# IlzeAmandaA/VAE-GP-ODE

Measured on AMD Instinct MI355X. Metric: latent_trajectories_per_sec, higher is better.
Workload: dtype f32; 1 GPU; configs[1]: ode1 DF q=6 M=100 S=256 T=16 batch=256; step = full ELBO training step (encoder, GP draw, rk4 rollout, decoder, ELBO, backward, Adam), L=1; global_batch=256, mc_draws=1, solver=rk4 (3/8 rule), parallelism=dp1, hip_graph=True, graph_scope=whole, gp_side_stream=True, batchnorm=per-process statistics

## Files before the change

vae-gp-ode_amd/csrc/conv_mfma.hpp:

```cpp
#pragma once
#include <hip/hip_runtime.h>
#include <cstdint>
#include <type_traits>
#include "bn_math.hpp"
#include "bn_sink.hpp"

namespace gp {

typedef float f32x4 __attribute__((ext_vector_type(4)));

template <int N, class F> __device__ __forceinline__ void static_for(F&& f) {
  if constexpr (N > 0) {
    static_for<N - 1>(f);
    f(std::integral_constant<int, N - 1>{});
  }
}

#ifdef CONVT_PROBE
__device__ unsigned long long g_probe[8];
#define PROBE_T(v) const long long v = clock64()
#define PROBE_ADD(i, v) do { if (threadIdx.x == 0 && blockIdx.x == 0) g_probe[i] += (unsigned long long)(clock64() - (v)); } while (0)
#else
#define PROBE_T(v)
#define PROBE_ADD(i, v)
#endif

constexpr int cmax_(int a, int b) { return a > b ? a : b; }
constexpr int plane_stride_unit(int n) { return ((n + 15) / 32) * 32 + 16; }

template <class L, int NCS_> struct FwdPolicy {
  static constexpr int KC = L::CI, NC = L::CO, NCS = NCS_, NCLS = L::S * L::S, KK = L::K * L::K;
  static constexpr int SH = L::HI, OH = L::HO, HP = L::HP, PADL = L::PL;
  static constexpr int PS = plane_stride_unit(HP * HP);
  static constexpr int WROW = NCS;
  static constexpr int WSLAB = KK * KC * WROW;
  static constexpr int NWE = KC * NCS * KK;
  static constexpr int class_tap_offset(int cls) {
    int off = 0;
    for (int c = 0; c < cls; ++c) off += ((L::K - c / L::S + L::S - 1) / L::S) * ((L::K - c % L::S + L::S - 1) / L::S);
    return off;
  }
  template <int CLS> struct C {
    static constexpr int py = CLS / L::S, px = CLS % L::S;
    static constexpr int nty = (L::K - py + L::S - 1) / L::S, ntx = (L::K - px + L::S - 1) / L::S, ntaps = nty * ntx;
    static constexpr int qy0 = cmax_(0, (L::P - py + L::S - 1) / L::S), qx0 = cmax_(0, (L::P - px + L::S - 1) / L::S);
    static constexpr int ny = (L::HO - 1 + L::P - py) / L::S - qy0 + 1, nx = (L::HO - 1 + L::P - px) / L::S - qx0 + 1;
    static constexpr int npc = ny * nx;
    static constexpr int slab_taps = class_tap_offset(CLS);
    static __device__ __forceinline__ int tap_off(int t) { return -(t / ntx) * HP - t % ntx; }
    static __device__ __forceinline__ int pix_addr(int p) { return (qy0 + p / nx + PADL) * HP + qx0 + p % nx + PADL; }
    static constexpr __host__ __device__ int out_off(int p) {
      return (L::S * (qy0 + p / nx) + py - L::P) * OH + L::S * (qx0 + p % nx) + px - L::P;
    }
  };
  static __device__ __forceinline__ size_t w_src(int e, int n0) {
    const int ci = e / (NCS * KK), r = e % (NCS * KK);
    return ((size_t)ci * NC + n0) * KK + r;
  }
  static __device__ __forceinline__ int w_dst(int e) {
    const int ci = e / (NCS * KK), r = e % (NCS * KK), col = r / KK, ky = (r % KK) / L::K, kx = r % L::K;
    const int py = ky % L::S, px = kx % L::S;
    int off = 0;
    for (int c = 0; c < py * L::S + px; ++c) off += ((L::K - c / L::S + L::S - 1) / L::S) * ((L::K - c % L::S + L::S - 1) / L::S);
    const int tap = (ky / L::S) * ((L::K - px + L::S - 1) / L::S) + kx / L::S;
    return ((off + tap) * KC + ci) * WROW + col;
  }
};

template <class L, int NCS_> struct BwdDataPolicy {
  static constexpr int KC = L::CO, NC = L::CI, NCS = NCS_, NCLS = 1, KK = L::K * L::K;
  static constexpr int SH = L::HO, OH = L::HI, HP = L::GP_, PADL = L::P;
  static constexpr int PS = L::S == 1 ? plane_stride_unit(HP * HP) : (HP * HP) | 1;
  static constexpr int WROW = NCS;
  static constexpr int WSLAB = KK * KC * WROW;
  static constexpr int NWE = KC * NCS * KK;
  template <int CLS> struct C {
    static constexpr int ntaps = KK, ntx = L::K, npc = L::HI * L::HI, nx = L::HI, slab_taps = 0;
    static __device__ __forceinline__ int tap_off(int t) { return (t / L::K) * HP + t % L::K; }
    static __device__ __forceinline__ int pix_addr(int p) { return L::S * (p / nx) * HP + L::S * (p % nx); }
    static constexpr __host__ __device__ int out_off(int p) { return p; }
  };
  static __device__ __forceinline__ size_t w_src(int e, int n0) { return (size_t)n0 * KC * KK + e; }
  static __device__ __forceinline__ int w_dst(int e) {
    const int cil = e / (KC * KK), co = (e / KK) % KC, tap = e % KK;
    return (tap * KC + co) * WROW + cil;
  }
};

template <class PL> constexpr bool igemm_tf_in_pad() { return PL::PS % 4 == 0 && (PL::HP * PL::HP + 3) / 4 * 4 + 4 <= PL::PS; }

template <class CG, int NG, int TG, int NCJ, int KC, int WROW, int PS, int KBMAX = 8>
__device__ __forceinline__ void igemm_tile_mma(const float* __restrict__ s_img, const float* __restrict__ sw, const int (&abase)[TG],
                                               int lk, int lr, f32x4 (&acc)[TG][NCJ]) {
  constexpr int KB = (KC / 4) < KBMAX ? (KC / 4) : KBMAX;
  constexpr int NB = KC / (4 * KB);
  constexpr int nsteps = CG::ntaps * NB;
  float bfA[KB][NCJ], afA[KB][NG], bfB[KB][NCJ], afB[KB][NG];
  auto fetch = [&](int s, float (&bf)[KB][NCJ], float (&af)[KB][NG]) {
    const int t = s / NB, cb = (s % NB) * 4 * KB;
    const float* wp = sw + ((size_t)t * KC + cb + lk) * WROW + lr;
    const int ao = CG::tap_off(t) + cb * PS;
#pragma unroll
    for (int kk = 0; kk < KB; ++kk) {
#pragma unroll
      for (int c = 0; c < NCJ; ++c) bf[kk][c] = wp[4 * kk * WROW + c * 16];
#pragma unroll
      for (int g = 0; g < NG; ++g) af[kk][g] = s_img[abase[g] + ao + 4 * kk * PS];
    }
  };
  auto mma = [&](const float (&bf)[KB][NCJ], const float (&af)[KB][NG]) {
#pragma unroll
    for (int kk = 0; kk < KB; ++kk)
#pragma unroll
      for (int g = 0; g < NG; ++g)
#pragma unroll
        for (int c = 0; c < NCJ; ++c)
          acc[g][c] = __builtin_amdgcn_mfma_f32_16x16x4f32(bf[kk][c], af[kk][g], acc[g][c], 0, 0, 0);
  };
  fetch(0, bfA, afA);
  int s = 0;
  if constexpr (KBMAX < 8) {
#pragma nounroll
    while (true) {
      if (s + 1 < nsteps) fetch(s + 1, bfB, afB);
      mma(bfA, afA);
      if (++s >= nsteps) break;
      if (s + 1 < nsteps) fetch(s + 1, bfA, afA);
      mma(bfB, afB);
      if (++s >= nsteps) break;
    }
  } else {
    while (true) {
      if (s + 1 < nsteps) fetch(s + 1, bfB, afB);
      mma(bfA, afA);
      if (++s >= nsteps) break;
      if (s + 1 < nsteps) fetch(s + 1, bfA, afA);
      mma(bfB, afB);
      if (++s >= nsteps) break;
    }
  }
}

extern __shared__ __attribute__((aligned(16))) float igemm_smem[];

template <class PL, int IPB, int TG, int NCJ, bool PAIR, int NTHR, bool DB = false, bool PC = false, bool STATS = false>
__global__ __launch_bounds__(NTHR, NTHR == 256 ? 2 : 1) void k_conv_igemm(const float* __restrict__ x, const float* __restrict__ w,
                                                      const float* __restrict__ bias, float* __restrict__ y, int B,
                                                      const float* __restrict__ in_bn, BnSink sink) {
  constexpr int KC = PL::KC, NC = PL::NC, NCS = PL::NCS, NCLS = PL::NCLS, SH = PL::SH, OH = PL::OH, HP = PL::HP, PS = PL::PS;
  constexpr int PADL = PL::PADL, WROW = PL::WROW, NWE = PL::NWE;
  static_assert(NCS % 16 == 0 && NC % NCS == 0 && KC % 4 == 0 && NTHR % 256 == 0, "MFMA tiling");
  static_assert(!PC || (NTHR == 768 && DB), "producer / consumer form: 8 + 4 wavefronts on double-buffered planes");
  constexpr int NW = PC ? 8 : NTHR / 64;
  constexpr int PT = PC ? 256 : NTHR;
  constexpr int KBM = PC ? 4 : 8;
  constexpr int NCO = NCS / 16;
  static_assert(NCO % NCJ == 0, "channel tiles per job");
  constexpr int NJ = NCO / NCJ;
  static_assert(NJ == 1 || TG == 1, "tile groups share all channel tiles");
  static_assert(!STATS || NJ == 1, "output statistics: a lane keeps the same channels in every job of a pass");
  constexpr int IMG = KC * PS;
  static_assert(IMG % 4 == 0, "float4 zero fill");
  constexpr int SRC = KC * SH * SH;
  static_assert(SRC % 4 == 0, "float4 source fetch");
  constexpr int NLD = (IPB * SRC / 4 + PT - 1) / PT;
  constexpr int NBUF = DB ? 2 : 1;
  float* s_img = igemm_smem;
  float* s_w = igemm_smem + NBUF * IPB * IMG;
  constexpr int TFO = (HP * HP + 3) / 4 * 4;
  constexpr bool TF_PAD = igemm_tf_in_pad<PL>();
  float* s_sm = s_w + PL::WSLAB + (TF_PAD ? 0 : 4 * KC);
  float4* s_tf_tail = reinterpret_cast<float4*>(s_w + PL::WSLAB);
  auto tf_slot = [&](int ch) -> float4* { return TF_PAD ? reinterpret_cast<float4*>(s_img + ch * PS + TFO) : s_tf_tail + ch; };
  const int tid = threadIdx.x, lane = tid & 63, wave = __builtin_amdgcn_readfirstlane(tid >> 6);
  const int lr = lane & 15, lk = lane >> 4;
  const int ptid = PC ? tid - 512 : tid;
  const int ngroups = (B + IPB - 1) / IPB;
  const float4* x4 = reinterpret_cast<const float4*>(x);
  const int jw = (wave & 3) * (NW / 4) + (wave >> 2);

  PROBE_T(pt_all);
  for (int e = tid; e < NBUF * IPB * IMG / 4; e += NTHR) reinterpret_cast<float4*>(s_img)[e] = float4{0.f, 0.f, 0.f, 0.f};
  if (in_bn) {
    if (TF_PAD) __syncthreads();
    for (int e = tid; e < KC; e += NTHR) *tf_slot(e) = reinterpret_cast<const float4*>(in_bn)[e];
  }
  if (STATS)
    for (int e = tid; e < 2 * NC; e += NTHR) s_sm[e] = 0.f;

  constexpr int NPASS = NC / NCS;
  const bool spread = NPASS > 1 && gridDim.x % NPASS == 0;
  const int gstride = spread ? gridDim.x / NPASS : gridDim.x;
  const int gfirst = spread ? blockIdx.x % gstride : blockIdx.x;
  for (int pass = spread ? blockIdx.x / gstride : 0; pass < (spread ? blockIdx.x / gstride + 1 : NPASS); ++pass) {
    const int n0 = pass * NCS;
    __syncthreads();
    PROBE_T(pt_w);
    for (int base = 0; base < NWE; base += NTHR * 8) {
      float v[8];
#pragma unroll
      for (int u = 0; u < 8; ++u) {
        const int e = base + tid + NTHR * u;
        v[u] = e < NWE ? w[PL::w_src(e, n0)] : 0.f;
      }
#pragma unroll
      for (int u = 0; u < 8; ++u) {
        const int e = base + tid + NTHR * u;
        if (e < NWE) s_w[PL::w_dst(e)] = v[u];
      }
    }
    PROBE_ADD(0, pt_w);

    float kshift[NCJ][4], bs[NCJ][4], bq[NCJ][4];
#pragma unroll
    for (int cc = 0; cc < NCJ; ++cc)
#pragma unroll
      for (int r = 0; r < 4; ++r) {
        kshift[cc][r] = STATS ? bn_sink_shift(sink, n0 + cc * 16 + 4 * lk + r) : 0.f;
        bs[cc][r] = bq[cc][r] = 0.f;
      }
    float4 pre[NLD];
    auto prefetch = [&](int grp) __attribute__((always_inline)) {
      const int b0 = grp * IPB;
      const int nf4 = min(IPB, B - b0) * (SRC / 4);
      const float4* src = x4 + (size_t)b0 * (SRC / 4);
#pragma unroll
      for (int i = 0; i < NLD; ++i) {
        const int f = ptid + PT * i;
        if (PC) pre[i] = src[min(f, nf4 - 1)];
        else if (f < nf4) pre[i] = src[f];
      }
    };
    auto scatter = [&](float* __restrict__ img, int nimg) __attribute__((always_inline)) {
      const int nf4 = nimg * (SRC / 4);
#pragma unroll
      for (int i = 0; i < NLD; ++i) {
        const int f = ptid + PT * i;
        if (f < nf4) {
          const float v[4] = {pre[i].x, pre[i].y, pre[i].z, pre[i].w};
          int pl = (4 * f) / (SH * SH), q = (4 * f) % (SH * SH), row = q / SH, col = q % SH;
#pragma unroll
          for (int k = 0; k < 4; ++k) {
            img[pl * PS + (row + PADL) * HP + col + PADL] = in_bn ? bn_relu(v[k], *tf_slot(pl % KC)) : v[k];
            if (SH % 4 != 0 || k < 3) {
              if (++col == SH) { col = 0; if (++row == SH) { row = 0; ++pl; } }
            }
          }
        }
      }
    };
    auto jobs = [&](const float* __restrict__ img, int b0, int nimg, int pf_grp = -1) {
      PROBE_T(pt_rng);
      int wtot = 0;
      constexpr int NCG = PAIR ? NCLS / 2 : NCLS;
      static_for<NCG>([&](auto c) {
        constexpr int c0 = PAIR ? 2 * decltype(c)::value : decltype(c)::value;
        using G0 = typename PL::template C<c0>;
        using G1 = typename PL::template C<PAIR ? c0 + 1 : c0>;
        wtot += ((nimg * G0::npc + 15) / 16) * NJ * (G0::ntaps + (PAIR ? G1::ntaps : 0));
      });
      const int lo = (wtot * jw) / NW, hi = (wtot * (jw + 1)) / NW;
      int cbase = 0;
      PROBE_ADD(0, pt_rng);
      static_for<NCG>([&](auto c) {
        constexpr int c0 = PAIR ? 2 * decltype(c)::value : decltype(c)::value;
        using G = typename PL::template C<c0>;
        using G1 = typename PL::template C<PAIR ? c0 + 1 : c0>;
        static_assert(!PAIR || (G::npc == G1::npc && G::nx == G1::nx), "paired classes cover the same pixel grid");
        static_assert(!PAIR || (G::out_off(0) == G1::out_off(0) + 1 && G::out_off(G::npc - 1) == G1::out_off(G::npc - 1) + 1 &&
                                G1::out_off(0) % 2 == 0 && OH % 2 == 0), "paired classes write neighbouring, 8-byte aligned columns");
        constexpr int ntaps = G::ntaps + (PAIR ? G1::ntaps : 0), npc = G::npc;
        const float* swc = s_w + G::slab_taps * KC * WROW;
        const float* swc1 = s_w + G1::slab_taps * KC * WROW;
        const int mtot = nimg * npc;
        const int njobs = ((mtot + 15) / 16) * NJ;
        const int nlo = lo - cbase - ntaps / 2, nhi = hi - cbase - ntaps / 2;
        const int ub = min(njobs, nlo <= 0 ? 0 : (nlo + ntaps - 1) / ntaps), ue = min(njobs, nhi <= 0 ? 0 : (nhi + ntaps - 1) / ntaps);
        cbase += njobs * ntaps;
        for (int u0 = ub; u0 < ue; u0 += TG) {
          PROBE_T(pt_su);
          const int ng = min(TG, ue - u0);
          const int t0 = u0 / NJ, jc = u0 % NJ;
          int abase[TG], abase1[TG];
#pragma unroll
          for (int g = 0; g < TG; ++g) {
            int m = (t0 + g) * 16 + lr;
            m = (g < ng && m < mtot) ? m : 0;
            const int im = m / npc, p = m % npc;
            abase[g] = im * IMG + lk * PS + G::pix_addr(p);
            abase1[g] = im * IMG + lk * PS + G1::pix_addr(p);
          }
          f32x4 acc[TG][NCJ], acc1[TG][NCJ];
#pragma unroll
          for (int g = 0; g < TG; ++g)
#pragma unroll
            for (int cc = 0; cc < NCJ; ++cc) acc[g][cc] = acc1[g][cc] = f32x4{0.f, 0.f, 0.f, 0.f};
          float bv[NCJ][4];
#pragma unroll
          for (int cc = 0; cc < NCJ; ++cc)
#pragma unroll
            for (int r = 0; r < 4; ++r) bv[cc][r] = bias ? bias[n0 + (jc * NCJ + cc) * 16 + 4 * lk + r] : 0.f;
          PROBE_ADD(6, pt_su);
          PROBE_T(pt_mm);
          auto run = [&](auto gtag, const float* sw, const int (&ab)[TG], f32x4 (&ac)[TG][NCJ]) {
            using GG = typename decltype(gtag)::type;
            switch (ng) {
              case 1: igemm_tile_mma<GG, 1, TG, NCJ, KC, WROW, PS, KBM>(img, sw, ab, lk, lr, ac); break;
              case 2: if constexpr (TG >= 2) igemm_tile_mma<GG, 2, TG, NCJ, KC, WROW, PS, KBM>(img, sw, ab, lk, lr, ac); break;
              case 3: if constexpr (TG >= 3) igemm_tile_mma<GG, 3, TG, NCJ, KC, WROW, PS, KBM>(img, sw, ab, lk, lr, ac); break;
              default: if constexpr (TG >= 4) igemm_tile_mma<GG, 4, TG, NCJ, KC, WROW, PS, KBM>(img, sw, ab, lk, lr, ac); break;
            }
          };
          run(std::common_type<G>{}, swc + jc * NCJ * 16, abase, acc);
          if (pf_grp >= 0) { prefetch(pf_grp); pf_grp = -1; }
          if constexpr (PAIR) run(std::common_type<G1>{}, swc1 + jc * NCJ * 16, abase1, acc1);
          PROBE_ADD(3, pt_mm);
          PROBE_T(pt_st);
#pragma unroll
          for (int g = 0; g < TG; ++g) {
            const int m = (t0 + g) * 16 + lr;
            if (g < ng && m < mtot) {
              const int im = m / npc, p = m % npc;
              const int ch0 = n0 + jc * NCJ * 16 + 4 * lk;
              float* yp = y + ((size_t)(b0 + im) * NC + ch0) * (OH * OH) + (PAIR ? G1::out_off(p) : G::out_off(p));
#pragma unroll
              for (int cc = 0; cc < NCJ; ++cc)
#pragma unroll
                for (int r = 0; r < 4; ++r) {
                  const float v0 = acc[g][cc][r] + bv[cc][r];
                  if constexpr (PAIR) {
                    const float v1 = acc1[g][cc][r] + bv[cc][r];
                    *reinterpret_cast<float2*>(yp + (size_t)(cc * 16 + r) * (OH * OH)) = float2{v1, v0};
                    if (STATS) { const float d = v1 - kshift[cc][r]; bs[cc][r] += d; bq[cc][r] = fmaf(d, d, bq[cc][r]); }
                  } else {
                    yp[(size_t)(cc * 16 + r) * (OH * OH)] = v0;
                  }
                  if (STATS) { const float d = v0 - kshift[cc][r]; bs[cc][r] += d; bq[cc][r] = fmaf(d, d, bq[cc][r]); }
                }
            }
          }
          PROBE_ADD(4, pt_st);
        }
      });
      if (pf_grp >= 0) prefetch(pf_grp);
    };
    if constexpr (PC) {
      const bool producer = wave >= 8;
      int cur = 0;
      if (producer) {
        __builtin_amdgcn_s_setprio(3);
        if (gfirst < ngroups) prefetch(gfirst);
      }
      __syncthreads();
      if (producer) {
        if (gfirst < ngroups) scatter(s_img, min(IPB, B - gfirst * IPB));
        if (gfirst + gstride < ngroups) prefetch(gfirst + gstride);
      }
      __syncthreads();
      for (int grp = gfirst; grp < ngroups; grp += gstride) {
        const int b0 = grp * IPB, nxt = grp + gstride;
        if (producer) {
          if (nxt < ngroups) {
            scatter(s_img + (cur ^ 1) * (IPB * IMG), min(IPB, B - nxt * IPB));
            if (nxt + gstride < ngroups) prefetch(nxt + gstride);
          }
        } else {
          jobs(s_img + cur * (IPB * IMG), b0, min(IPB, B - b0));
        }
        __syncthreads();
        cur ^= 1;
      }
    } else if constexpr (!DB) {
      if (gfirst < ngroups) prefetch(gfirst);
      for (int grp = gfirst; grp < ngroups; grp += gstride) {
        const int b0 = grp * IPB;
        const int nimg = min(IPB, B - b0);
        PROBE_T(pt_b1);
        __syncthreads();
        PROBE_ADD(1, pt_b1);
        PROBE_T(pt_sc);
        scatter(s_img, nimg);
        __syncthreads();
        PROBE_ADD(2, pt_sc);
        PROBE_T(pt_pf);
        PROBE_ADD(7, pt_pf);
        jobs(s_img, b0, nimg, grp + gstride < ngroups ? grp + gstride : -1);
      }
    } else {
      const bool early = wave < NW / 2;
      int cur = 0;
      if (gfirst < ngroups) prefetch(gfirst);
      __syncthreads();
      if (gfirst < ngroups) scatter(s_img, min(IPB, B - gfirst * IPB));
      if (gfirst + gstride < ngroups) prefetch(gfirst + gstride);
      __syncthreads();
      for (int grp = gfirst; grp < ngroups; grp += gstride) {
        const int b0 = grp * IPB, nxt = grp + gstride;
        const int nimg = min(IPB, B - b0);
        float* bc = s_img + cur * (IPB * IMG);
        float* bn = s_img + (cur ^ 1) * (IPB * IMG);
        if (early && nxt < ngroups) {
          scatter(bn, min(IPB, B - nxt * IPB));
          if (nxt + gstride < ngroups) prefetch(nxt + gstride);
        }
        jobs(bc, b0, nimg);
        if (!early && nxt < ngroups) {
          scatter(bn, min(IPB, B - nxt * IPB));
          if (nxt + gstride < ngroups) prefetch(nxt + gstride);
        }
        __syncthreads();
        cur ^= 1;
      }
    }
    if constexpr (STATS) {
      __syncthreads();
      float* red = s_w;
#pragma unroll
      for (int cc = 0; cc < NCJ; ++cc)
#pragma unroll
        for (int r = 0; r < 4; ++r) {
          const float a = row_allreduce16(bs[cc][r]), b = row_allreduce16(bq[cc][r]);
          if (lr == 0 && wave < NW) {
            red[(wave * NCS + cc * 16 + 4 * lk + r) * 2] = a;
            red[(wave * NCS + cc * 16 + 4 * lk + r) * 2 + 1] = b;
          }
        }
      __syncthreads();
      if (tid < 2 * NCS) {
        float t = 0.f;
        for (int wv = 0; wv < NW; ++wv) t += red[wv * NCS * 2 + tid];
        s_sm[2 * n0 + tid] = t;
      }
    }
  }
  if constexpr (STATS) {
    __syncthreads();
    bn_sink_publish<NC, NTHR>(sink, s_sm);
  }
  PROBE_ADD(5, pt_all);
}

constexpr int pad2mod4(int n) { return n + ((2 - n % 4) + 4) % 4; }

template <class L> struct WgradGeo {
  static constexpr int NPIX = L::HI * L::HI, NKS = (NPIX + 3) / 4;
  static constexpr int PSX = pad2mod4(NKS * 4);
  static constexpr int GP = L::GP_;
  static constexpr int GPH = L::S == 2 ? (GP + 1) / 2 : GP;
  static constexpr int HPL = GP * GPH;
  static constexpr int PSG = pad2mod4(L::S == 2 ? 2 * HPL : HPL);
  static constexpr int IMGX = L::CI * PSX, IMGG = L::CO * PSG;
  static_assert(L::S == 1 || L::S == 2, "stride");
};

template <class L, int IPB, int WM, int WN, int WT, bool PIPE, bool HAS_BN, int NTHR>
// ... 206 lines not shown
```

vae-gp-ode_amd/csrc/vae_conv_tiled.hip:

```cpp
#include <hip/hip_runtime.h>
#include <cstdlib>
#include <cstdint>
#include "gp_launch.hpp"
#include <type_traits>
#include "conv_layers.hpp"
#include "conv_mfma.hpp"
#include "conv_dec10_mfma.hpp"
#include "conv_dec1_mfma.hpp"
#include "conv_dec4_mfma.hpp"

namespace gp {



extern __shared__ __attribute__((aligned(16))) float tsm[];

template <class L, int IPB>
__global__ __launch_bounds__(256) void k_convT_fwd(const float* __restrict__ x, const float* __restrict__ w,
                                                    const float* __restrict__ bias, float* __restrict__ y, int B) {
  constexpr int CI = L::CI, CO = L::CO, HI = L::HI, HO = L::HO, HP = L::HP, K = L::K, S = L::S, P = L::P, PL = L::PL;
  constexpr int CPT = CO % 16 == 0 ? 16 : 8;
  static_assert(CO % CPT == 0, "8 or 16 output channels per thread");
  constexpr int NG = CO / CPT;
  constexpr int IMG = CI * HP * HP;
// ... 219 lines not shown
    const int ox0 = seg * 4;
    float acc[4] = {bv, bv, bv, bv};
    const float* img = s_img + im * IMG;
#pragma unroll 2
    for (int ci = 0; ci < CI; ++ci) {
#pragma unroll
      for (int ky = 0; ky < 5; ++ky) {
        const float4* rp = reinterpret_cast<const float4*>(img + (ci * WP + (oy + 4 - ky)) * WP + ox0);
        const float4 a = rp[0], b = rp[1];
        const float v[8] = {a.x, a.y, a.z, a.w, b.x, b.y, b.z, b.w};
        const float4 w4 = *reinterpret_cast<const float4*>(s_w + (ci * 5 + ky) * 8);
        const float w5 = s_w[(ci * 5 + ky) * 8 + 4];
        const float wk[5] = {w4.x, w4.y, w4.z, w4.w, w5};
#pragma unroll
        for (int j = 0; j < 4; ++j)
#pragma unroll
          for (int kx = 0; kx < 5; ++kx) acc[j] = fmaf(v[j + 4 - kx], wk[kx], acc[j]);
      }
    }
    *reinterpret_cast<float4*>(y + ((size_t)(b0 + im) * H + oy) * H + ox0) = make_float4(acc[0], acc[1], acc[2], acc[3]);
  }
}

__global__ __launch_bounds__(256) void k_dec10_wgrad(const float* __restrict__ x, const float* __restrict__ gy,
                                                      float* __restrict__ part, int B, int b_per_split) {
  constexpr int CI = 16, H = 28, NP = H * H, XS = NP + 1, GW = 32;
  float* s_x = tsm;
  float* s_g = tsm + CI * XS;
  const int tid = threadIdx.x, ci = tid & 15, pl = tid >> 4;
  const int b0 = blockIdx.x * b_per_split, b1 = min(B, b0 + b_per_split);
  float acc[25];
#pragma unroll
  for (int t = 0; t < 25; ++t) acc[t] = 0.f;
  for (int b = b0; b < b1; ++b) {
    __syncthreads();
    for (int e = tid; e < CI * NP; e += 256) s_x[(e / NP) * XS + e % NP] = x[(size_t)b * CI * NP + e];
    for (int e = tid; e < GW * GW; e += 256) {
      const int yy = e / GW - 2, xx = e % GW - 2;
      s_g[e] = (yy >= 0 && yy < H && xx >= 0 && xx < H) ? gy[(size_t)b * NP + yy * H + xx] : 0.f;
    }
    __syncthreads();
    for (int p = pl; p < NP; p += 16) {
      const int iy = p / H, ix = p % H;
      const float xv = s_x[ci * XS + p];
      const float* gp = s_g + iy * GW + ix;
#pragma unroll
      for (int ky = 0; ky < 5; ++ky)
#pragma unroll
        for (int kx = 0; kx < 5; ++kx) acc[ky * 5 + kx] = fmaf(xv, gp[ky * GW + kx], acc[ky * 5 + kx]);
    }
  }
  __syncthreads();
  float* s_red = tsm;
#pragma unroll
  for (int t = 0; t < 25; ++t) s_red[(pl * 16 + ci) * 25 + t] = acc[t];
  __syncthreads();
  for (int e = tid; e < CI * 25; e += 256) {
    float v = 0.f;
    for (int l = 0; l < 16; ++l) v += s_red[l * 400 + e];
    part[(size_t)blockIdx.x * 400 + e] = v;
  }
}

__global__ void k_sum_splits_t(const float* __restrict__ part, int nsplit, size_t n, float* __restrict__ out) {
  const size_t e = (size_t)blockIdx.x * blockDim.x + threadIdx.x;
  if (e >= n) return;
  float acc = 0.f;
  for (int s = 0; s < nsplit; ++s) acc += part[(size_t)s * n + e];
  out[e] = acc;
}

template <class L> static bool matches(int Ci_conv, int Co_conv, int H, int Ho, int K, int S, int P) {
  return Ci_conv == L::CO && Co_conv == L::CI && H == L::HO && Ho == L::HI && K == L::K && S == L::S && P == L::P;
}

static bool use_mfma() {
  static int v = -1;
  if (v < 0) { const char* e = getenv("GPODE_CONV_VALU"); v = (e && e[0] == '1') ? 0 : 1; }
  return v == 1;
}

constexpr int kSinkMaxWg = 512;

template <class PL, int IPB, int TG, int NCJ, bool PAIR = false, int NTHR = 512, bool DB = false, bool PC = false, bool STATS = false>
static int launch_igemm(const float* x, const float* w, const float* bias, float* y, int B, hipStream_t st, const char* what,
                        const float* in_bn = nullptr, const BnSink* sink = nullptr) {
  constexpr size_t lds = igemm_lds_bytes<PL, IPB, DB, STATS>();
  static_assert(lds <= (NTHR >= 512 ? 160 : 80) * 1024, "LDS budget");
  auto km = k_conv_igemm<PL, IPB, TG, NCJ, PAIR, NTHR, DB, PC, STATS>;
  if (set_max_lds((const void*)km, lds)) return 1;
  const int ngroups = (B + IPB - 1) / IPB;
  const int cap = num_cus() * (NTHR >= 512 ? 1 : 2);
  if (STATS && cap > kSinkMaxWg) return set_error("%s: more workgroups than the statistics scratch holds", what);
  hipLaunchKernelGGL(km, ngroups < cap ? ngroups : cap, NTHR, lds, st, x, w, bias, y, B, in_bn, STATS ? *sink : BnSink{});
  return check_launch(what);
}

static bool conv_pc_enabled() {
  static const bool on = [] { const char* e = getenv("GPODE_CONV_PC"); return e && e[0] == '1'; }();
  return on;
}

template <class L, int IPB, int IPBM, int COS>
static int launch_T1(const float* x, const float* w, const float* bias, float* y, int B, hipStream_t st, const float* in_bn,
                     const BnSink* sink = nullptr) {
  constexpr int MAXTAPS = ((L::K + L::S - 1) / L::S) * ((L::K + L::S - 1) / L::S);
  const size_t lds = sizeof(float) * ((size_t)IPB * L::CI * L::HP * L::HP + (size_t)MAXTAPS * L::CI * L::CO);
  if (use_mfma() && (reinterpret_cast<uintptr_t>(x) & 15) == 0) {
    constexpr int TG = COS >= 64 ? 1 : (COS >= 32 ? 2 : 4);
    constexpr bool PAIR = L::S == 2 && (L::HO % 2 == 0) && (L::P % 2 == 1);
    if constexpr (std::is_same<L, Dec7>::value) {
      static const bool db = [] { const char* e = getenv("GPODE_DEC7_FWD_DB"); return e && e[0] == '1'; }();
      if (db) return launch_igemm<FwdPolicy<L, COS>, 1, TG, COS / 16, PAIR, 512, true>(x, w, bias, y, B, st, "convT_fwd_mfma", in_bn);
      if (conv_pc_enabled() && B > 2 * num_cus() && !sink)
        return launch_igemm<FwdPolicy<L, COS>, 1, 2, COS / 16, PAIR, 768, true, true>(x, w, bias, y, B, st, "convT_fwd_mfma_pc", in_bn);
    }
    if (sink) return launch_igemm<FwdPolicy<L, COS>, IPBM, TG, COS / 16, PAIR, 512, false, false, true>(x, w, bias, y, B, st, "convT_fwd_mfma_stats", in_bn, sink);
    return launch_igemm<FwdPolicy<L, COS>, IPBM, TG, COS / 16, PAIR>(x, w, bias, y, B, st, "convT_fwd_mfma", in_bn);
  }
  if (sink) return set_error("convT forward with output statistics needs the matrix-core path (16-byte aligned input, GPODE_CONV_VALU unset)");
  if (in_bn) return set_error("convT forward with a fused BatchNorm input needs the matrix-core path (16-byte aligned input, GPODE_CONV_VALU unset)");
  auto kern = k_convT_fwd<L, IPB>;
  if (set_max_lds((const void*)kern, lds)) return 1;
  hipLaunchKernelGGL(kern, (B + IPB - 1) / IPB, 256, lds, st, x, w, bias, y, B);
  return check_launch("convT_fwd_tiled");
}

template <class L, int IPB, int COC, int IPBM, int CIS, int TG, int NCJ, int NTHR = 512>
static int launch_T2(const float* gy, const float* w, float* gx, int B, hipStream_t st) {
  if constexpr (IPBM > 0) {
    if (use_mfma() && (reinterpret_cast<uintptr_t>(gy) & 15) == 0)
      return launch_igemm<BwdDataPolicy<L, CIS>, IPBM, TG, NCJ, false, NTHR>(gy, w, nullptr, gx, B, st, "convT_bwd_data_mfma");
  }
  const size_t lds = sizeof(float) * ((size_t)IPB * L::CO * L::GP_ * L::GP_ + (size_t)COC * L::K * L::K * L::CI);
  auto kern = k_convT_bwd_data<L, IPB, COC>;
  if (set_max_lds((const void*)kern, lds)) return 1;
  hipLaunchKernelGGL(kern, (B + IPB - 1) / IPB, 256, lds, st, gy, w, gx, B);
  return check_launch("convT_bwd_data_tiled");
}

template <class L, int IPBM, int WM, int WN, int WT, bool PIPE>
static int launch_wgrad_mfma(const float* x, const float* gy, float* gw, float* scratch, int B, hipStream_t st, const float* in_bn) {
  constexpr int NTHR = WM * WN * WT * 64;
  constexpr size_t ldsm = wgrad_lds_bytes<L, IPBM>();
  static_assert(ldsm <= (NTHR == 512 ? 160 : 80) * 1024, "LDS budget");
  auto km = k_convT_wgrad_mfma<L, IPBM, WM, WN, WT, PIPE, false, NTHR>;
  auto kb = k_convT_wgrad_mfma<L, IPBM, WM, WN, WT, PIPE, true, NTHR>;
  if (set_max_lds((const void*)km, ldsm) || set_max_lds((const void*)kb, ldsm)) return 1;
  const int ngroups = (B + IPBM - 1) / IPBM;
  const int cap = num_cus() * (512 / NTHR);
  const int nwg = ngroups < cap ? ngroups : cap;
  if (in_bn) hipLaunchKernelGGL(kb, nwg, NTHR, ldsm, st, x, gy, scratch, B, in_bn);
  else hipLaunchKernelGGL(km, nwg, NTHR, ldsm, st, x, gy, scratch, B, in_bn);
  const size_t n = (size_t)L::CI * L::CO * L::K * L::K;
  if (reduce_job(RedJob{scratch, gw, nwg, (int)n, 1, L::CI / 16, L::CO / 16, L::K * L::K}, st)) return 1;
  return check_launch("convT_wgrad_mfma");
}

int wgrad_v2_dec7(const float* x, const float* gy, float* gw, float* scratch, int B, hipStream_t st, const float* in_bn);
int wgrad_v2_dec4(const float* x, const float* gy, float* gw, float* scratch, int B, hipStream_t st, const float* in_bn);
static bool wgrad_v2_enabled() {
  static const bool off = [] { const char* e = getenv("GPODE_WGRAD_V1"); return e && e[0] == '1'; }();
  return !off && use_mfma();
}

template <class L, int COW, int IPBM, int WM, int WN, int WT, bool PIPE>
static int launch_T3(const float* x, const float* gy, float* gw, float* scratch, int B, hipStream_t st, const float* in_bn) {
  if (use_mfma() && ((reinterpret_cast<uintptr_t>(x) | reinterpret_cast<uintptr_t>(gy)) & 15) == 0)
    return launch_wgrad_mfma<L, IPBM, WM, WN, WT, PIPE>(x, gy, gw, scratch, B, st, in_bn);
  if (in_bn) return set_error("convT weight gradient with a fused BatchNorm input needs the matrix-core path");
  constexpr int NT = L::CI * (COW / 4), PSPLIT = 256 / NT, KK = L::K * L::K;
  size_t fl = (size_t)L::HI * L::HI * L::CI + (size_t)L::GP_ * L::GP_ * COW;
  const size_t red = PSPLIT > 1 ? (size_t)PSPLIT * NT * KK * 4 : 0;
  if (red > fl) fl = red;
  const size_t lds = sizeof(float) * fl;
  int nsplit = B < 256 ? B : 256;
  const int bps = (B + nsplit - 1) / nsplit;
  nsplit = (B + bps - 1) / bps;
  auto kern = k_convT_wgrad<L, COW>;
  if (set_max_lds((const void*)kern, lds)) return 1;
  hipLaunchKernelGGL(kern, dim3(nsplit, L::CO / COW), 256, lds, st, x, gy, scratch, B, bps);
  const size_t n = (size_t)L::CI * L::CO * KK;
  if (reduce_job(RedJob{scratch, gw, nsplit, (int)n, 0, 0, 0, 0}, st)) return 1;
  return check_launch("convT_wgrad_tiled");
}


int tiled_bwd_data(const float* gy, const float* w, const float* bias, float* gx, int B, int Ci, int H, int W, int Co, int K, int S,
                   int P, int Ho, int Wo, const float* in_bn, hipStream_t st, const BnSink* sink) {
  if (H != W || Ho != Wo) return -1;
  if (sink && !(use_mfma() && (matches<Dec7>(Ci, Co, H, Ho, K, S, P) || matches<Dec4>(Ci, Co, H, Ho, K, S, P) ||
                               (matches<Dec1>(Ci, Co, H, Ho, K, S, P) && !in_bn))))
    return set_error("gpode_convT_fwd_stats: no specialisation for this geometry");
  if (matches<Dec7>(Ci, Co, H, Ho, K, S, P)) return launch_T1<Dec7, 3, 2, 16>(gy, w, bias, gx, B, st, in_bn, sink);
  if (matches<Dec4>(Ci, Co, H, Ho, K, S, P)) {
    static const int tapcols = [] { const char* e = getenv("GPODE_DEC4_TAPCOLS"); return e ? (e[0] == '1' ? 1 : 0) : -1; }();
    if ((tapcols == 1 || (tapcols < 0 && B <= 4 * num_cus())) && use_mfma()) {
      const size_t lds = sizeof(float) * (dec4::NPI * dec4::TLD + 4 * dec4::CI + (sink ? 2 * dec4::CO * dec4::NPO : 0));
      if (set_max_lds((const void*)dec4::k_fwd<true>, lds) || set_max_lds((const void*)dec4::k_fwd<false>, lds) ||
          set_max_lds((const void*)dec4::k_fwd<true, true>, lds) || set_max_lds((const void*)dec4::k_fwd<false, true>, lds)) return 1;
      const int nwg = B < num_cus() ? B : num_cus();
      const BnSink sk = sink ? *sink : BnSink{};
      if (sink && in_bn) hipLaunchKernelGGL((dec4::k_fwd<true, true>), nwg, 512, lds, st, gy, w, bias, gx, B, in_bn, sk);
      else if (sink) hipLaunchKernelGGL((dec4::k_fwd<false, true>), nwg, 512, lds, st, gy, w, bias, gx, B, in_bn, sk);
      else if (in_bn) hipLaunchKernelGGL((dec4::k_fwd<true>), nwg, 512, lds, st, gy, w, bias, gx, B, in_bn, sk);
      else hipLaunchKernelGGL((dec4::k_fwd<false>), nwg, 512, lds, st, gy, w, bias, gx, B, in_bn, sk);
      return check_launch("dec4_fwd_tapcols");
    }
    return launch_T1<Dec4, 3, 2, 16>(gy, w, bias, gx, B, st, in_bn, sink);
  }
  if (matches<Dec1>(Ci, Co, H, Ho, K, S, P)) {
    static const bool old = [] { const char* e = getenv("GPODE_DEC1_ENGINE"); return e && e[0] == '1'; }();
    if (!in_bn && use_mfma() && (!old || sink)) {
      const size_t lds = sizeof(float) * 2 * dec1::NPI * dec1::TLD;
      if (set_max_lds((const void*)dec1::k_fwd<false>, lds) || set_max_lds((const void*)dec1::k_fwd<true>, lds)) return 1;
      const int cap = 2 * num_cus();
      if (sink) hipLaunchKernelGGL(dec1::k_fwd<true>, B < cap ? B : cap, 256, lds, st, gy, w, bias, gx, B, *sink);
      else hipLaunchKernelGGL(dec1::k_fwd<false>, B < cap ? B : cap, 256, lds, st, gy, w, bias, gx, B, BnSink{});
      return check_launch("dec1_fwd_mfma");
    }
    return launch_T1<Dec1, 8, 8, 64>(gy, w, bias, gx, B, st, in_bn);
  }
  if (matches<Enc3>(Ci, Co, H, Ho, K, S, P) && !in_bn && B >= 96) {
    constexpr int IPB = 2;
    constexpr int MAXTAPS = ((Enc3::K + Enc3::S - 1) / Enc3::S) * ((Enc3::K + Enc3::S - 1) / Enc3::S);
    const size_t lds = sizeof(float) * ((size_t)IPB * Enc3::CI * Enc3::HP * Enc3::HP + (size_t)MAXTAPS * Enc3::CI * Enc3::CO);
    auto kern = k_convT_fwd<Enc3, IPB>;
    if (set_max_lds((const void*)kern, lds)) return 1;
    hipLaunchKernelGGL(kern, (B + IPB - 1) / IPB, 256, lds, st, gy, w, bias, gx, B);
    return check_launch("enc_conv3_bwd_data_tiled");
  }
  if (matches<Enc6>(Ci, Co, H, Ho, K, S, P) && use_mfma() && (reinterpret_cast<uintptr_t>(gy) & 15) == 0)
  {
    static const bool ipb8 = [] { const char* e = getenv("GPODE_ENC6_IPB8"); return e && e[0] == '1'; }();
    if (!ipb8 && B < 4 * num_cus()) return launch_igemm<FwdPolicy<Enc6, 16>, 2, 4, 1>(gy, w, bias, gx, B, st, "enc_conv6_bwd_data_mfma", in_bn);
    return launch_igemm<FwdPolicy<Enc6, 16>, 8, 4, 1>(gy, w, bias, gx, B, st, "enc_conv6_bwd_data_mfma", in_bn);
  }
  if (matches<Dec10>(Ci, Co, H, Ho, K, S, P)) {
    if (use_mfma()) {
      const size_t ldsm = sizeof(float) * dec10::KK * dec10::PST;
      if (set_max_lds((const void*)dec10::k_fwd<true>, ldsm) || set_max_lds((const void*)dec10::k_fwd<false>, ldsm)) return 1;
      if (in_bn) hipLaunchKernelGGL(dec10::k_fwd<true>, B < num_cus() ? B : num_cus(), 512, ldsm, st, gy, w, bias, gx, B, in_bn);
      else hipLaunchKernelGGL(dec10::k_fwd<false>, B < num_cus() ? B : num_cus(), 512, ldsm, st, gy, w, bias, gx, B, in_bn);
      return check_launch("dec10_fwd_mfma");
    }
    constexpr int IPB = 2;
    const size_t lds = sizeof(float) * ((size_t)IPB * 16 * 32 * 32 + 16 * 5 * 8);
    auto kern = k_dec10_fwd<IPB>;
    if (set_max_lds((const void*)kern, lds)) return 1;
    hipLaunchKernelGGL(kern, (B + IPB - 1) / IPB, 256, lds, st, gy, w, bias, gx, B);
    return check_launch("dec10_fwd");
  }
  return -1;
}

int tiled_fwd(const float* x, const float* w, const float* bias, float* y, int B, int Ci, int H, int W, int Co, int K, int S, int P,
              int Ho, int Wo, hipStream_t st) {
  if (H != W || Ho != Wo) return -1;
  if (use_mfma() && (reinterpret_cast<uintptr_t>(x) & 15) == 0) {
    if (matches<Enc3>(Ci, Co, H, Ho, K, S, P)) return launch_igemm<BwdDataPolicy<Enc3, 16>, 4, 4, 1>(x, w, bias, y, B, st, "enc_conv3_fwd_mfma");
    if (matches<Enc6>(Ci, Co, H, Ho, K, S, P)) return launch_igemm<BwdDataPolicy<Enc6, 32>, 8, 1, 2>(x, w, bias, y, B, st, "enc_conv6_fwd_mfma");
  }
  if (bias) return -1;
  if (matches<Dec7>(Ci, Co, H, Ho, K, S, P)) return launch_T2<Dec7, 2, 8, 1, 16, 2, 1, 256>(x, w, y, B, st);
  if (matches<Dec4>(Ci, Co, H, Ho, K, S, P)) {
    static const bool alt = [] { const char* e = getenv("GPODE_DEC4_BWD_3IMG"); return e && e[0] == '1'; }();
    if (alt) return launch_T2<Dec4, 3, 8, 3, 16, 1, 1>(x, w, y, B, st);
    return launch_T2<Dec4, 3, 8, 2, 32, 1, 1>(x, w, y, B, st);
  }
  if (matches<Dec1>(Ci, Co, H, Ho, K, S, P)) {
    static const bool old = [] { const char* e = getenv("GPODE_DEC1_ENGINE"); return e && e[0] == '1'; }();
    if (use_mfma() && !old && (reinterpret_cast<uintptr_t>(x) & 15) == 0) {
      const size_t lds = sizeof(float) * (2 * dec1::GYF + 4 * dec1::NPI * 33);
      const int cap = 2 * num_cus();
      hipLaunchKernelGGL(dec1::k_bwd_data, B < cap ? B : cap, 256, lds, st, x, w, y, B);
      return check_launch("dec1_bwd_data_mfma");
    }
    return launch_T2<Dec1, 8, 32, 6, 32, 1, 1>(x, w, y, B, st);
  }

  if (matches<Dec10>(Ci, Co, H, Ho, K, S, P)) {
    if (use_mfma() && (reinterpret_cast<uintptr_t>(x) & 15) == 0) {
      constexpr int IPB = 8;
      const size_t ldsm = sizeof(float) * IPB * dec10::PLANE;
      const int ngroups = (B + IPB - 1) / IPB;
      hipLaunchKernelGGL(dec10::k_bwd_data<IPB>, ngroups < num_cus() ? ngroups : num_cus(), 512, ldsm, st, x, w, y, B);
      return check_launch("dec10_bwd_data_mfma");
    }
    return launch_T2<Dec10, 1, 1, 0, 16, 1, 1>(x, w, y, B, st);
  }
  return -1;
}

constexpr int kDec10BnMaxWg = 512;
int dec10_bn_scratch_floats() { return 2 * kDec10BnMaxWg * dec10::CI * 2; }

__global__ __launch_bounds__(512) void k_dec10_parts_reduce(const float* __restrict__ part, int nsplit, float* __restrict__ out, int stride2) {
  __shared__ float sA[dec10::CI], sB[dec10::CI];
  dec10::reduce_parts(part, nsplit, sA, sB);
  __syncthreads();
  const int tid = threadIdx.x;
  if (stride2) { if (tid < 2 * dec10::CI) out[tid] = (tid & 1 ? sB : sA)[tid >> 1]; }
  else if (tid < dec10::CI) out[tid] = sA[tid];
}

template <int IPB, int MODE, bool WGRAD = false, typename... A>
static int launch_dec10_bn(int B, hipStream_t st, A... args) {
  const size_t lds = sizeof(float) * ((size_t)IPB * dec10::PLANE + 8 * 4 * dec10::CI * 2 + 2 * dec10::CI + (WGRAD ? 8 * dec10::CI * 32 : 0));
  auto kern = dec10::k_bwd_data_bn<IPB, MODE, WGRAD>;
  if (set_max_lds((const void*)kern, lds)) return 1;
  const int ngroups = (B + IPB - 1) / IPB, cap = 2 * num_cus() < kDec10BnMaxWg ? 2 * num_cus() : kDec10BnMaxWg;
  hipLaunchKernelGGL(kern, ngroups < cap ? ngroups : cap, 512, lds, st, args...);
  return 0;
}
static int dec10_bn_nwg(int B, int& ipb) {
  ipb = B >= 4 * num_cus() ? 4 : 2;
  const int ngroups = (B + ipb - 1) / ipb, cap = 2 * num_cus() < kDec10BnMaxWg ? 2 * num_cus() : kDec10BnMaxWg;
  return ngroups < cap ? ngroups : cap;
}

int dec10_bn_wgrad_scratch_floats() { return kDec10BnMaxWg * dec10::CI * dec10::KK + kDec10BnMaxWg; }
int dec10_bn_bwd_sums(const float* c, const float* gy, const float* w, const float* gamma, const float* beta, const float* mean,
                      const float* invstd, float* sums, int B, float* scratch, hipStream_t st, float* gw, float* wscratch, float* gbias) {
  if (((reinterpret_cast<uintptr_t>(gy) | reinterpret_cast<uintptr_t>(c)) & 15) != 0) return set_error("gpode_dec10_bn_bwd_sums: c / gy must be 16-byte aligned");
  if (gw && !wscratch) return set_error("gpode_dec10_bn_bwd_sums_wgrad: scratch for the weight-gradient partials missing");
  int ipb;
  const int nwg = dec10_bn_nwg(B, ipb);
  float* np_ = nullptr;
  const float* cnp = nullptr;
  int rc;
  if (gw) {
    float* part_b = gbias ? wscratch + (size_t)kDec10BnMaxWg * dec10::CI * dec10::KK : nullptr;
    if (ipb == 4) rc = launch_dec10_bn<4, 0, true>(B, st, gy, w, c, gamma, beta, mean, invstd, B, scratch, 0, 0.f, cnp, cnp, 0, np_, np_, np_, np_, wscratch, part_b);
    else rc = launch_dec10_bn<2, 0, true>(B, st, gy, w, c, gamma, beta, mean, invstd, B, scratch, 0, 0.f, cnp, cnp, 0, np_, np_, np_, np_, wscratch, part_b);
    if (!rc) {
      const RedJob jobs[2] = {RedJob{wscratch, gw, nwg, dec10::CI * dec10::KK, 0, 0, 0, 0}, RedJob{part_b, gbias, nwg, 1, 0, 0, 0, 0}};
      if (reduce_jobs(jobs, gbias ? 2 : 1, st)) return 1;
    }
  } else if (ipb == 4) rc = launch_dec10_bn<4, 0>(B, st, gy, w, c, gamma, beta, mean, invstd, B, scratch, 0, 0.f, cnp, cnp, 0, np_, np_, np_, np_, np_, np_);
  else rc = launch_dec10_bn<2, 0>(B, st, gy, w, c, gamma, beta, mean, invstd, B, scratch, 0, 0.f, cnp, cnp, 0, np_, np_, np_, np_, np_, np_);
  if (rc) return rc;
  if (sums) hipLaunchKernelGGL(k_dec10_parts_reduce, 1, 512, 0, st, scratch, nwg, sums, 1);
  return check_launch("dec10_bn_bwd_sums");
}

int dec10_bn_bwd_apply(const float* c, const float* gy, const float* w, const float* gamma, const float* beta, const float* mean,
                       const float* invstd, const float* gathered, const float* wts, int W, float count_all, float* gc, float* ggamma,
// ... 68 lines not shown
```

Baseline: 97200 trajectories/s.

## Add producer/consumer MFMA kernel for Dec7 bwd-data and drop old PC path

Adds a new backward-data convolution kernel for the Dec7 layer, enabled by default when MFMA is available. It uses 768 threads, with 8 consumer waves that keep their weights in registers and 4 high-priority producer waves that stage incoming gradient images into a triple-buffered LDS ring. Consumers walk pixel windows that can span image boundaries and use a fixed-distance register prefetch with scheduling barriers, aiming to overlap global loads with matrix-core work. The previous opt-in producer/consumer variant of the generic implicit-GEMM kernel is removed. The cost is a new code path with heavy register use, one workgroup per CU, and a __syncthreads per window.

```diff
diff --git a/vae-gp-ode_amd/csrc/conv_bwd_v2.hpp b/vae-gp-ode_amd/csrc/conv_bwd_v2.hpp
--- /dev/null
+++ b/vae-gp-ode_amd/csrc/conv_bwd_v2.hpp
@@ -0,0 +1,123 @@
+#pragma once
+#include "conv_mfma.hpp"
+
+namespace gp {
+
+template <class L> struct BdV2 {
+  using PL = BwdDataPolicy<L, L::CI>;
+  static constexpr int KC = L::CO, NC = L::CI, KK = L::K * L::K;
+  static constexpr int NCT = NC / 16;
+  static constexpr int NKS = KK * (KC / 4);
+  static constexpr int NPX = L::HI * L::HI;
+  static constexpr int SRC = KC * L::HO * L::HO;
+  static constexpr int PS = PL::PS, HP = PL::HP, IMG = KC * PS;
+  static constexpr int NBUF = 3, NCW = 8, NTHR = 768, NLT = NTHR - 64 * NCW;
+  static constexpr int TPW = 2;
+  static constexpr int WIN = 16 * 4 * TPW;
+  static constexpr int PF = 2;
+  static_assert(NCT * 4 == NCW, "the two consumers of a SIMD split the output channels");
+  static_assert(KC % 4 == 0 && L::HO % 4 == 0 && SRC % 4 == 0, "float4 rows of the source");
+  static_assert(WIN <= NPX, "a window touches at most two images");
+  static constexpr int koff(int s) { return (s / (KC / 4)) / L::K * HP + (s / (KC / 4)) % L::K + (s % (KC / 4)) * 4 * PS; }
+  static_assert(4 * koff(NKS - 1) < 65536, "operand offsets fit the ds_read immediate");
+  static constexpr size_t lds_bytes() { return sizeof(float) * (size_t)NBUF * IMG; }
+};
+
+template <class E, int NT>
+__device__ __forceinline__ void bdv2_tiles(const float* __restrict__ s_buf, const int (&base)[E::TPW], const float (&wr)[E::NKS],
+                                           f32x4 (&acc)[E::TPW]) {
+  float bf[E::PF + 1][NT];
+  auto fetch = [&](auto sc) {
+    constexpr int s = decltype(sc)::value;
+#pragma unroll
+    for (int t = 0; t < NT; ++t) bf[s % (E::PF + 1)][t] = s_buf[base[t] + E::koff(s)];
+  };
+#pragma unroll
+  for (int t = 0; t < NT; ++t) acc[t] = f32x4{0.f, 0.f, 0.f, 0.f};
+  static_for<E::PF>([&](auto sc) { fetch(sc); });
+  static_for<E::NKS>([&](auto sc) {
+    constexpr int s = decltype(sc)::value;
+    if constexpr (s + E::PF < E::NKS) fetch(std::integral_constant<int, s + E::PF>{});
+    __builtin_amdgcn_sched_barrier(0);
+#pragma unroll
+    for (int t = 0; t < NT; ++t) acc[t] = __builtin_amdgcn_mfma_f32_16x16x4f32(wr[s], bf[s % (E::PF + 1)][t], acc[t], 0, 0, 0);
+    __builtin_amdgcn_sched_barrier(0);
+  });
+}
+
+template <class L>
+__global__ __launch_bounds__(768) void k_conv_bwd_data_v2(const float* __restrict__ gy, const float* __restrict__ w, float* __restrict__ gx,
+                                                          int B) {
+  using E = BdV2<L>;
+  using PL = typename E::PL;
+  constexpr int KC = E::KC, NC = E::NC, KK = E::KK, NPX = E::NPX, IMG = E::IMG, PS = E::PS, HP = E::HP, WIN = E::WIN, NKS = E::NKS;
+  constexpr int HO = L::HO, P = L::P, NLT = E::NLT;
+  float* s_buf = igemm_smem;
+  const int tid = threadIdx.x, lane = tid & 63, wave = __builtin_amdgcn_readfirstlane(tid >> 6);
+  const int nit = ((int)blockIdx.x < B) ? (B - 1 - (int)blockIdx.x) / (int)gridDim.x + 1 : 0;
+  const int npx = nit * NPX, nwin = (npx + WIN - 1) / WIN;
+  auto last_img = [&](int i) { return min(nit - 1, (i * WIN + WIN - 1) / NPX); };
+
+  for (int e = tid; e < E::NBUF * IMG / 4; e += E::NTHR) reinterpret_cast<float4*>(s_buf)[e] = float4{0.f, 0.f, 0.f, 0.f};
+  __syncthreads();
+
+  if (wave >= E::NCW) {
+    __builtin_amdgcn_s_setprio(3);
+    const int lt = tid - 64 * E::NCW;
+    constexpr int N4 = E::SRC / 4, NLD = (N4 + NLT - 1) / NLT;
+    auto stage = [&](int j) __attribute__((always_inline)) {
+      const float4* src = reinterpret_cast<const float4*>(gy) + (size_t)((int)blockIdx.x + j * (int)gridDim.x) * N4;
+      float* buf = s_buf + (j % E::NBUF) * IMG;
+      float4 v[NLD];
+#pragma unroll
+      for (int i = 0; i < NLD; ++i) v[i] = src[min(lt + NLT * i, N4 - 1)];
+#pragma unroll
+      for (int i = 0; i < NLD; ++i) {
+        const int f = lt + NLT * i;
+        const int pl = (4 * f) / (HO * HO), q = (4 * f) % (HO * HO), row = q / HO, col = q % HO;
+        float* d = buf + pl * PS + (row + P) * HP + col + P;
+        if (f < N4) { d[0] = v[i].x; d[1] = v[i].y; d[2] = v[i].z; d[3] = v[i].w; }
+      }
+    };
+    if (nit > 0) stage(0);
+    __syncthreads();
+    for (int i = 0; i < nwin; ++i) {
+      if (i + 1 < nwin && last_img(i + 1) > last_img(i)) stage(last_img(i + 1));
+      __syncthreads();
+    }
+    return;
+  }
+
+  const int lr = lane & 15, lk = lane >> 4, ct = wave >> 2, sm = wave & 3;
+  float wr[NKS];
+#pragma unroll
+  for (int s = 0; s < NKS; ++s) wr[s] = w[((size_t)(16 * ct + lr) * KC + 4 * (s % (KC / 4)) + lk) * KK + s / (KC / 4)];
+  __syncthreads();
+  for (int i = 0; i < nwin; ++i) {
+    const int t0 = i * WIN + 16 * sm;
+    int base[E::TPW], mm[E::TPW];
+#pragma unroll
+    for (int t = 0; t < E::TPW; ++t) {
+      mm[t] = t0 + 64 * t + lr;
+      const int m = min(mm[t], npx - 1);
+      const int j = m / NPX, p = m - j * NPX;
+      base[t] = (j % E::NBUF) * IMG + lk * PS + PL::template C<0>::pix_addr(p);
+    }
+    f32x4 acc[E::TPW];
+    int nt = 0;
+    if (t0 + 64 < npx) { bdv2_tiles<E, 2>(s_buf, base, wr, acc); nt = 2; }
+    else if (t0 < npx) { bdv2_tiles<E, 1>(s_buf, base, wr, acc); nt = 1; }
+#pragma unroll
+    for (int t = 0; t < E::TPW; ++t) {
+      if (t < nt && mm[t] < npx) {
+        const int j = mm[t] / NPX, p = mm[t] - j * NPX;
+        float* o = gx + ((size_t)((int)blockIdx.x + j * (int)gridDim.x) * NC + 16 * ct + 4 * lk) * NPX + p;
+#pragma unroll
+        for (int r = 0; r < 4; ++r) o[(size_t)r * NPX] = acc[t][r];
+      }
+    }
+    __syncthreads();
+  }
+}
+
+}
diff --git a/vae-gp-ode_amd/csrc/conv_mfma.hpp b/vae-gp-ode_amd/csrc/conv_mfma.hpp
--- a/vae-gp-ode_amd/csrc/conv_mfma.hpp
+++ b/vae-gp-ode_amd/csrc/conv_mfma.hpp
@@ -89,10 +89,10 @@
 
 template <class PL> constexpr bool igemm_tf_in_pad() { return PL::PS % 4 == 0 && (PL::HP * PL::HP + 3) / 4 * 4 + 4 <= PL::PS; }
 
-template <class CG, int NG, int TG, int NCJ, int KC, int WROW, int PS, int KBMAX = 8>
+template <class CG, int NG, int TG, int NCJ, int KC, int WROW, int PS>
 __device__ __forceinline__ void igemm_tile_mma(const float* __restrict__ s_img, const float* __restrict__ sw, const int (&abase)[TG],
                                                int lk, int lr, f32x4 (&acc)[TG][NCJ]) {
-  constexpr int KB = (KC / 4) < KBMAX ? (KC / 4) : KBMAX;
+  constexpr int KB = (KC / 4) < 8 ? (KC / 4) : 8;
   constexpr int NB = KC / (4 * KB);
   constexpr int nsteps = CG::ntaps * NB;
   float bfA[KB][NCJ], afA[KB][NG], bfB[KB][NCJ], afB[KB][NG];
@@ -119,41 +119,27 @@
   };
   fetch(0, bfA, afA);
   int s = 0;
-  if constexpr (KBMAX < 8) {
-#pragma nounroll
-    while (true) {
-      if (s + 1 < nsteps) fetch(s + 1, bfB, afB);
-      mma(bfA, afA);
-      if (++s >= nsteps) break;
-      if (s + 1 < nsteps) fetch(s + 1, bfA, afA);
-      mma(bfB, afB);
-      if (++s >= nsteps) break;
-    }
-  } else {
-    while (true) {
-      if (s + 1 < nsteps) fetch(s + 1, bfB, afB);
-      mma(bfA, afA);
-      if (++s >= nsteps) break;
-      if (s + 1 < nsteps) fetch(s + 1, bfA, afA);
-      mma(bfB, afB);
-      if (++s >= nsteps) break;
-    }
+  while (true) {
+    if (s + 1 < nsteps) fetch(s + 1, bfB, afB);
+    mma(bfA, afA);
+    if (++s >= nsteps) break;
+    if (s + 1 < nsteps) fetch(s + 1, bfA, afA);
+    mma(bfB, afB);
+    if (++s >= nsteps) break;
   }
 }
 
 extern __shared__ __attribute__((aligned(16))) float igemm_smem[];
 
-template <class PL, int IPB, int TG, int NCJ, bool PAIR, int NTHR, bool DB = false, bool PC = false, bool STATS = false>
+template <class PL, int IPB, int TG, int NCJ, bool PAIR, int NTHR, bool DB = false, bool STATS = false>
 __global__ __launch_bounds__(NTHR, NTHR == 256 ? 2 : 1) void k_conv_igemm(const float* __restrict__ x, const float* __restrict__ w,
                                                       const float* __restrict__ bias, float* __restrict__ y, int B,
                                                       const float* __restrict__ in_bn, BnSink sink) {
   constexpr int KC = PL::KC, NC = PL::NC, NCS = PL::NCS, NCLS = PL::NCLS, SH = PL::SH, OH = PL::OH, HP = PL::HP, PS = PL::PS;
   constexpr int PADL = PL::PADL, WROW = PL::WROW, NWE = PL::NWE;
   static_assert(NCS % 16 == 0 && NC % NCS == 0 && KC % 4 == 0 && NTHR % 256 == 0, "MFMA tiling");
-  static_assert(!PC || (NTHR == 768 && DB), "producer / consumer form: 8 + 4 wavefronts on double-buffered planes");
-  constexpr int NW = PC ? 8 : NTHR / 64;
-  constexpr int PT = PC ? 256 : NTHR;
-  constexpr int KBM = PC ? 4 : 8;
+  constexpr int NW = NTHR / 64;
+  constexpr int PT = NTHR;
   constexpr int NCO = NCS / 16;
   static_assert(NCO % NCJ == 0, "channel tiles per job");
   constexpr int NJ = NCO / NCJ;
@@ -174,7 +160,7 @@
   auto tf_slot = [&](int ch) -> float4* { return TF_PAD ? reinterpret_cast<float4*>(s_img + ch * PS + TFO) : s_tf_tail + ch; };
   const int tid = threadIdx.x, lane = tid & 63, wave = __builtin_amdgcn_readfirstlane(tid >> 6);
   const int lr = lane & 15, lk = lane >> 4;
-  const int ptid = PC ? tid - 512 : tid;
+  const int ptid = tid;
   const int ngroups = (B + IPB - 1) / IPB;
   const float4* x4 = reinterpret_cast<const float4*>(x);
   const int jw = (wave & 3) * (NW / 4) + (wave >> 2);
@@ -227,8 +213,7 @@
 #pragma unroll
       for (int i = 0; i < NLD; ++i) {
         const int f = ptid + PT * i;
-        if (PC) pre[i] = src[min(f, nf4 - 1)];
-        else if (f < nf4) pre[i] = src[f];
+        if (f < nf4) pre[i] = src[f];
       }
     };
     auto scatter = [&](float* __restrict__ img, int nimg) __attribute__((always_inline)) {
@@ -305,10 +290,10 @@
           auto run = [&](auto gtag, const float* sw, const int (&ab)[TG], f32x4 (&ac)[TG][NCJ]) {
             using GG = typename decltype(gtag)::type;
             switch (ng) {
-              case 1: igemm_tile_mma<GG, 1, TG, NCJ, KC, WROW, PS, KBM>(img, sw, ab, lk, lr, ac); break;
-              case 2: if constexpr (TG >= 2) igemm_tile_mma<GG, 2, TG, NCJ, KC, WROW, PS, KBM>(img, sw, ab, lk, lr, ac); break;
-              case 3: if constexpr (TG >= 3) igemm_tile_mma<GG, 3, TG, NCJ, KC, WROW, PS, KBM>(img, sw, ab, lk, lr, ac); break;
-              default: if constexpr (TG >= 4) igemm_tile_mma<GG, 4, TG, NCJ, KC, WROW, PS, KBM>(img, sw, ab, lk, lr, ac); break;
+              case 1: igemm_tile_mma<GG, 1, TG, NCJ, KC, WROW, PS>(img, sw, ab, lk, lr, ac); break;
+              case 2: if constexpr (TG >= 2) igemm_tile_mma<GG, 2, TG, NCJ, KC, WROW, PS>(img, sw, ab, lk, lr, ac); break;
+              case 3: if constexpr (TG >= 3) igemm_tile_mma<GG, 3, TG, NCJ, KC, WROW, PS>(img, sw, ab, lk, lr, ac); break;
+              default: if constexpr (TG >= 4) igemm_tile_mma<GG, 4, TG, NCJ, KC, WROW, PS>(img, sw, ab, lk, lr, ac); break;
             }
           };
           run(std::common_type<G>{}, swc + jc * NCJ * 16, abase, acc);
@@ -344,33 +329,7 @@
       });
       if (pf_grp >= 0) prefetch(pf_grp);
     };
-    if constexpr (PC) {
-      const bool producer = wave >= 8;
-      int cur = 0;
-      if (producer) {
-        __builtin_amdgcn_s_setprio(3);
-        if (gfirst < ngroups) prefetch(gfirst);
-      }
-      __syncthreads();
-      if (producer) {
-        if (gfirst < ngroups) scatter(s_img, min(IPB, B - gfirst * IPB));
-        if (gfirst + gstride < ngroups) prefetch(gfirst + gstride);
-      }
-      __syncthreads();
-      for (int grp = gfirst; grp < ngroups; grp += gstride) {
-        const int b0 = grp * IPB, nxt = grp + gstride;
-        if (producer) {
-          if (nxt < ngroups) {
-            scatter(s_img + (cur ^ 1) * (IPB * IMG), min(IPB, B - nxt * IPB));
-            if (nxt + gstride < ngroups) prefetch(nxt + gstride);
-          }
-        } else {
-          jobs(s_img + cur * (IPB * IMG), b0, min(IPB, B - b0));
-        }
-        __syncthreads();
-        cur ^= 1;
-      }
-    } else if constexpr (!DB) {
+    if constexpr (!DB) {
       if (gfirst < ngroups) prefetch(gfirst);
       for (int grp = gfirst; grp < ngroups; grp += gstride) {
         const int b0 = grp * IPB;
diff --git a/vae-gp-ode_amd/csrc/vae_conv_tiled.hip b/vae-gp-ode_amd/csrc/vae_conv_tiled.hip
--- a/vae-gp-ode_amd/csrc/vae_conv_tiled.hip
+++ b/vae-gp-ode_amd/csrc/vae_conv_tiled.hip
@@ -325,23 +325,18 @@
 
 constexpr int kSinkMaxWg = 512;
 
-template <class PL, int IPB, int TG, int NCJ, bool PAIR = false, int NTHR = 512, bool DB = false, bool PC = false, bool STATS = false>
+template <class PL, int IPB, int TG, int NCJ, bool PAIR = false, int NTHR = 512, bool DB = false, bool STATS = false>
 static int launch_igemm(const float* x, const float* w, const float* bias, float* y, int B, hipStream_t st, const char* what,
                         const float* in_bn = nullptr, const BnSink* sink = nullptr) {
   constexpr size_t lds = igemm_lds_bytes<PL, IPB, DB, STATS>();
   static_assert(lds <= (NTHR >= 512 ? 160 : 80) * 1024, "LDS budget");
-  auto km = k_conv_igemm<PL, IPB, TG, NCJ, PAIR, NTHR, DB, PC, STATS>;
+  auto km = k_conv_igemm<PL, IPB, TG, NCJ, PAIR, NTHR, DB, STATS>;
   if (set_max_lds((const void*)km, lds)) return 1;
   const int ngroups = (B + IPB - 1) / IPB;
   const int cap = num_cus() * (NTHR >= 512 ? 1 : 2);
   if (STATS && cap > kSinkMaxWg) return set_error("%s: more workgroups than the statistics scratch holds", what);
   hipLaunchKernelGGL(km, ngroups < cap ? ngroups : cap, NTHR, lds, st, x, w, bias, y, B, in_bn, STATS ? *sink : BnSink{});
   return check_launch(what);
-}
-
-static bool conv_pc_enabled() {
-  static const bool on = [] { const char* e = getenv("GPODE_CONV_PC"); return e && e[0] == '1'; }();
-  return on;
 }
 
 template <class L, int IPB, int IPBM, int COS>
@@ -355,10 +350,8 @@
     if constexpr (std::is_same<L, Dec7>::value) {
       static const bool db = [] { const char* e = getenv("GPODE_DEC7_FWD_DB"); return e && e[0] == '1'; }();
       if (db) return launch_igemm<FwdPolicy<L, COS>, 1, TG, COS / 16, PAIR, 512, true>(x, w, bias, y, B, st, "convT_fwd_mfma", in_bn);
-      if (conv_pc_enabled() && B > 2 * num_cus() && !sink)
-        return launch_igemm<FwdPolicy<L, COS>, 1, 2, COS / 16, PAIR, 768, true, true>(x, w, bias, y, B, st, "convT_fwd_mfma_pc", in_bn);
-    }
-    if (sink) return launch_igemm<FwdPolicy<L, COS>, IPBM, TG, COS / 16, PAIR, 512, false, false, true>(x, w, bias, y, B, st, "convT_fwd_mfma_stats", in_bn, sink);
+    }
+    if (sink) return launch_igemm<FwdPolicy<L, COS>, IPBM, TG, COS / 16, PAIR, 512, false, true>(x, w, bias, y, B, st, "convT_fwd_mfma_stats", in_bn, sink);
     return launch_igemm<FwdPolicy<L, COS>, IPBM, TG, COS / 16, PAIR>(x, w, bias, y, B, st, "convT_fwd_mfma", in_bn);
   }
   if (sink) return set_error("convT forward with output statistics needs the matrix-core path (16-byte aligned input, GPODE_CONV_VALU unset)");
@@ -497,6 +490,12 @@
   return -1;
 }
 
+int conv_v2_dec7_bwd_data(const float* gy, const float* w, float* gx, int B, hipStream_t st);
+static bool conv_v2_enabled() {
+  static const bool off = [] { const char* e = getenv("GPODE_CONV_V1"); return e && e[0] == '1'; }();
+  return !off && use_mfma();
+}
+
 int tiled_fwd(const float* x, const float* w, const float* bias, float* y, int B, int Ci, int H, int W, int Co, int K, int S, int P,
               int Ho, int Wo, hipStream_t st) {
   if (H != W || Ho != Wo) return -1;
@@ -505,7 +504,10 @@
     if (matches<Enc6>(Ci, Co, H, Ho, K, S, P)) return launch_igemm<BwdDataPolicy<Enc6, 32>, 8, 1, 2>(x, w, bias, y, B, st, "enc_conv6_fwd_mfma");
   }
   if (bias) return -1;
-  if (matches<Dec7>(Ci, Co, H, Ho, K, S, P)) return launch_T2<Dec7, 2, 8, 1, 16, 2, 1, 256>(x, w, y, B, st);
+  if (matches<Dec7>(Ci, Co, H, Ho, K, S, P)) {
+    if (conv_v2_enabled() && (reinterpret_cast<uintptr_t>(x) & 15) == 0) return conv_v2_dec7_bwd_data(x, w, y, B, st);
+    return launch_T2<Dec7, 2, 8, 1, 16, 2, 1, 256>(x, w, y, B, st);
+  }
   if (matches<Dec4>(Ci, Co, H, Ho, K, S, P)) {
     static const bool alt = [] { const char* e = getenv("GPODE_DEC4_BWD_3IMG"); return e && e[0] == '1'; }();
     if (alt) return launch_T2<Dec4, 3, 8, 3, 16, 1, 1>(x, w, y, B, st);
diff --git a/vae-gp-ode_amd/csrc/vae_conv_v2.hip b/vae-gp-ode_amd/csrc/vae_conv_v2.hip
--- /dev/null
+++ b/vae-gp-ode_amd/csrc/vae_conv_v2.hip
@@ -0,0 +1,19 @@
+#include <hip/hip_runtime.h>
+#include <cstdint>
+#include "gp_launch.hpp"
+#include "conv_layers.hpp"
+#include "conv_bwd_v2.hpp"
+
+namespace gp {
+
+int conv_v2_dec7_bwd_data(const float* gy, const float* w, float* gx, int B, hipStream_t st) {
+  using E = BdV2<Dec7>;
+  constexpr size_t lds = E::lds_bytes();
+  static_assert(lds <= 160 * 1024, "LDS budget");
+  auto km = k_conv_bwd_data_v2<Dec7>;
+  if (set_max_lds((const void*)km, lds)) return 1;
+  hipLaunchKernelGGL(km, B < num_cus() ? B : num_cus(), E::NTHR, lds, st, gy, w, gx, B);
+  return check_launch("conv_v2_dec7_bwd_data");
+}
+
+}
```

Measured after the change: 101,600 trajectories/s (median of 6 runs). +4.5%, better.
